# Joseph-93/PhotoHive_DSP

Measured on AMD Instinct MI355X. Metric: images/sec (4000×3000 RGB8 full report) at 1/2/4/8 GPUs; HBM GB/s vs peak, higher is better.
Workload: dtype f64

## Files before the change

### photohive_dsp_amd/csrc/fft_ct.hip

```cpp
#include <algorithm>
#include <cstdlib>

#pragma clang fp contract(fast)

#include "fft_engine.h"
#include "phd_device.h"

namespace phd {

namespace {

using namespace fe;

typedef unsigned u32x4 __attribute__((ext_vector_type(4)));

constexpr double kWr = 0.299 / 255.0, kWg = 0.587 / 255.0, kWb = 0.114 / 255.0;

typedef unsigned u32x3a __attribute__((ext_vector_type(3), aligned(4)));
typedef const __attribute__((address_space(1))) u32x3a gu32x3a;
#ifndef PHD_ROW_NT
#define PHD_ROW_NT 0
#endif

__device__ __forceinline__ int byte_of(const u32x3a& w, int b) {
    const unsigned x = (b >> 2) == 0 ? w.x : ((b >> 2) == 1 ? w.y : w.z);
    return (x >> (8 * (b & 3))) & 255;
}

__device__ __forceinline__ u32x3a rot_px(const u32x3a& w, int r) {
    const int b = 3 * r, q = b >> 2, sh = b & 3;
    const unsigned l0 = q == 0 ? w.x : (q == 1 ? w.y : w.z);
    const unsigned l1 = q == 0 ? w.y : (q == 1 ? w.z : w.x);
    const unsigned l2 = q == 0 ? w.z : (q == 1 ? w.x : w.y);
    u32x3a o;
    o.x = __builtin_amdgcn_alignbyte(l1, l0, (unsigned)sh);
    o.y = __builtin_amdgcn_alignbyte(l2, l1, (unsigned)sh);
    o.z = __builtin_amdgcn_alignbyte(l0, l2, (unsigned)sh);
    return o;
}

template <int E, bool HFULL>
__device__ __forceinline__ void walk_runs(const double* __restrict__ lgb, int r0, int rend, const unsigned* rl,
                                          unsigned sg, unsigned long long* sl, double bscale,
                                          const double2* __restrict__ lt) {
    auto flush = [&](int k, double m, int e) {
        const double acc = fmax((double)e * 0.69314718055994530942 + log_mant(m, lt), 0.0);
        atomicAdd(&sl[k], bin_fixed(acc, bscale));
    };
    if (r0 >= rend) return;
    const int idx = (int)(sg & 255u);
    const unsigned chm = sg >> 8;
    if (__all(__popc(chm) <= 2)) {
        const int f1 = __builtin_ctz(chm | 0x80000000u), f2 = __builtin_ctz((chm & (chm - 1)) | 0x80000000u);
        double mp = 1.0, m0 = 1.0, m1 = 1.0;
        int es = 0, e0 = 0, e1 = 0;
#pragma unroll
        for (int j = 0; j < E; j++) {
            const int r = r0 + j;
            if (HFULL || r < rend) {
                const double pv = lgb[r];
                if (j > 0) {
                    const bool c1 = f1 == j, c2 = f2 == j;
                    m0 = c1 ? mp : m0;
                    e0 = c1 ? es : e0;
                    m1 = c2 ? mp : m1;
                    e1 = c2 ? es : e1;
                    mp = (c1 || c2) ? 1.0 : mp;
                    es = (c1 || c2) ? 0 : es;
                }
                int e;
                mp *= frexp(pv, &e);
                es += e;
            }
        }
        const int n = __popc(chm);
        flush(idx, n == 0 ? mp : m0, n == 0 ? es : e0);
        if (n >= 1) flush(idx + 1, n == 1 ? mp : m1, n == 1 ? es : e1);
        if (n == 2) flush(idx + 2, mp, es);
        return;
    }
    unsigned q1 = rl[idx + 1], q2 = rl[min(idx + 2, kColRunsMax - 1)], q3 = rl[min(idx + 3, kColRunsMax - 1)];
    int qi = idx + 4;
    int cur = idx, nxt = (int)(q1 >> 16);
    int esum = 0, n = 0, b0 = 0, b1 = 0, e0 = 0, e1 = 0;
    double mp = 1.0;
    double m0 = 1.0, m1 = 1.0;
    auto close = [&]() {
        if (n == 0) {
            b0 = cur; m0 = mp; e0 = esum; n = 1;
        } else if (n == 1) {
            b1 = cur; m1 = mp; e1 = esum; n = 2;
        } else {
            flush(cur, mp, esum);
        }
    };
#pragma unroll
    for (int j = 0; j < E; j++) {
        const int r = r0 + j;
        if (HFULL || r < rend) {
            const double pv = lgb[r];
            if (r >= nxt) {
                close();
                cur++;
                q1 = q2;
                q2 = q3;
                q3 = rl[min(qi++, kColRunsMax - 1)];
                nxt = (int)(q1 >> 16);
                mp = 1.0;
                esum = 0;
            }
            int e;
            mp *= frexp(pv, &e);
            esum += e;
        }
    }
    close();
    if (n > 0) flush(b0, m0, e0);
    if (n > 1) flush(b1, m1, e1);
}

template <int W, int T, int... Rs>
struct RowK {
    static constexpr int NTW = tw_entries<1, Rs...>();
    static constexpr int G4 = W / 4;
    static constexpr int LR = (G4 + T - 1) / T;
    static constexpr size_t lds = sizeof(double2) * (W + NTW);
    static_assert(W % 4 == 0, "row plans need W % 4 == 0");
    static_assert(Radices<Rs...>::product == W, "plan");
    static constexpr int BPC = (int)((160 * 1024) / lds) < 2 ? (int)((160 * 1024) / lds) : 2;
    static constexpr int MINW = (T >= 512 ? 4 : 2) * BPC / 2 > 0 ? (T >= 512 ? 4 : 2) * BPC / 2 : 1;
};

template <int W, int T, int... Rs>
__global__ __launch_bounds__(T, (RowK<W, T, Rs...>::MINW)) void k_rows_ct(const uint8_t* __restrict__ img, int H,
                                               const unsigned long long* __restrict__ sums,
                                               const double* __restrict__ k255g, const double2* __restrict__ twg,
                                               double2* __restrict__ inter, int ablate_arg,
                                               unsigned long long* __restrict__ rsum,
                                               const uint8_t* const* __restrict__ imgs, int nimg, long istride) {
    using K = RowK<W, T, Rs...>;
    const int ablate = PHD_ABL(ablate_arg);
    extern __shared__ __attribute__((aligned(16))) unsigned char smem[];
    double2* buf = reinterpret_cast<double2*>(smem);
    double2* tw = buf + W;
    const int tid = threadIdx.x;
    for (int i = tid; i < K::NTW; i += T) tw[i] = twg[i];
    const int P = (H + 1) / 2, G = (P + 3) / 4;
    const int x = blockIdx.x & 7, q = blockIdx.x >> 3, QA = gridDim.x >> 5;
    const int a = q >> 2, i4 = q & 3;
    auto item = [&](int s, int& im, int& pr) {
        const int m = x + 8 * (a + s * QA);
        im = m / G;
        pr = 4 * (m - im * G) + i4;
        return im < nimg && pr < P;
    };

    u32x3a rg[K::LR][2];
    auto fetch = [&](int im, int pr) {
        const int y0 = 2 * pr;
        const uint8_t* r0 = (imgs ? imgs[im] : img) + (size_t)y0 * 3 * W;
        const uint8_t* r1 = (y0 + 1 < H) ? r0 + 3 * W : r0;
#pragma unroll
        for (int j = 0; j < K::LR; j++) {
            const int g = (K::G4 % T == 0 || tid + j * T < K::G4) ? tid + j * T : 0;
#if PHD_ROW_NT
            rg[j][0] = __builtin_nontemporal_load((gu32x3a*)(r0 + 12 * g));
            rg[j][1] = __builtin_nontemporal_load((gu32x3a*)(r1 + 12 * g));
#else
            rg[j][0] = *(gu32x3a*)(r0 + 12 * g);
            rg[j][1] = *(gu32x3a*)(r1 + 12 * g);
#endif
        }
    };
    int s = 0, im = 0, pr = 0;
    bool live = item(0, im, pr);
    if (live) fetch(im, pr);
    __syncthreads();
    unsigned cs[3] = {0u, 0u, 0u};
    const int rot = (tid >> 1) & 3;
    constexpr int WF_ = W / 2 + 1, KP_ = (WF_ + 1) / 2, NSO_ = (4 * KP_ + T - 1) / T;
    {
        double2* slot = inter + (size_t)P * ct_row_stride(W) + (blockIdx.x & 63) * NSO_;
#pragma unroll
        for (int j = 0; j < NSO_; j++)
            if ((4 * KP_) % T == 0 || tid + j * T < 4 * KP_) slot[j] = make_double2(0.0, 0.0);
    }
    auto step = [&]() __attribute__((always_inline)) {
        const int y0 = 2 * pr;
        const bool two = y0 + 1 < H;
#pragma unroll
        for (int j = 0; j < K::LR; j++) {
            const int g = tid + j * T;
            if (K::G4 % T == 0 || g < K::G4) {
                double2 z[4];
                const u32x3a w0 = rot_px(rg[j][0], rot), w1 = rot_px(rg[j][1], rot);
#pragma unroll
                for (int e = 0; e < 4; e++) {
                    const double p0 = kWr * byte_of(w0, 3 * e) + kWg * byte_of(w0, 3 * e + 1) +
                                      kWb * byte_of(w0, 3 * e + 2);
                    const double p1 = kWr * byte_of(w1, 3 * e) + kWg * byte_of(w1, 3 * e + 1) +
                                      kWb * byte_of(w1, 3 * e + 2);
                    z[e] = make_double2(p0, two ? p1 : 0.0);
                    if (rsum) {
                        cs[0] += byte_of(w0, 3 * e) + (two ? byte_of(w1, 3 * e) : 0);
                        cs[1] += byte_of(w0, 3 * e + 1) + (two ? byte_of(w1, 3 * e + 1) : 0);
                        cs[2] += byte_of(w0, 3 * e + 2) + (two ? byte_of(w1, 3 * e + 2) : 0);
                    }
                }
#pragma unroll
                for (int e = 0; e < 4; e++) buf[4 * g + ((e + rot) & 3)] = z[e];
            }
        }
        int imn, prn;
        const bool next = item(s + 1, imn, prn);
        if (!(ablate & 4)) fetch(next ? imn : im, next ? prn : pr);
        __syncthreads();
        if (!(ablate & 1)) fft_lds<W, T, 1, Rs...>(buf, tw, tid);
        constexpr int WF = W / 2 + 1, KP = (WF + 1) / 2;
        double2* orow = inter + ((ablate & 8) ? (size_t)(blockIdx.x & 7) * ct_row_stride(W)
                                              : im * istride + (size_t)pr * ct_row_stride(W));
        constexpr int NSO = (4 * KP + T - 1) / T;
#pragma unroll
        for (int j = 0; j < NSO; j++) {
            const int i = tid + j * T;
            if ((4 * KP) % T == 0 || i < 4 * KP) {
                if (ablate & 2) continue;
                const int k = 2 * (i >> 2) + ((i >> 1) & 1);
                const bool second = i & 1;
                const int kk = k < WF ? k : 0;
                const int e = second ? (kk == 0 ? 0 : W - kk) : kk;
                const double* zp = reinterpret_cast<const double*>(buf + e);
                const double A = zp[second ? 1 : 0], B = zp[second ? 0 : 1];
                const double Ap = dpp_pair_swap(A), Bp = dpp_pair_swap(B);
                const double f = (k < WF && (two || !second)) ? 0.5 : 0.0;
                orow[i] = make_double2(f * (A + Bp), f * (B - Ap));
            }
        }
        __syncthreads();
        s++;
        im = imn;
        pr = prn;
        live = next;
    };
    while (live) step();
    if (rsum) {
        unsigned long long* red = reinterpret_cast<unsigned long long*>(smem);
        unsigned long long w3[3];
#pragma unroll
        for (int c = 0; c < 3; c++) w3[c] = wave_sum((unsigned long long)cs[c]);
        if (lane_id() == 0)
#pragma unroll
            for (int c = 0; c < 3; c++) red[(tid >> 6) * 3 + c] = w3[c];
        __syncthreads();
        if (tid < 3) {
            unsigned long long t = 0;
            for (int w = 0; w < T / 64; w++) t += red[w * 3 + tid];
            if (t) atomicAdd(&rsum[tid], t);
        }
    }
}

template <int H, int T, bool FULL, int... Rs>
struct ColK {
    using PL = Plan<H, T, 1, Rs...>;
    using L = typename PL::Last;
    static constexpr int R = L::OUT;
    static constexpr int NTW = tw_entries<1, Rs...>();
    static constexpr int P = (H + 1) / 2;
    static constexpr int CR = (2 * P + T - 1) / T;
    static constexpr int E = (H + T - 1) / T;
    static constexpr int RPT = (kColRunsMax + T - 1) / T;
    static constexpr size_t lds_base =
        sizeof(double2) * (H + NTW + kLogTab) + (sizeof(unsigned) + sizeof(unsigned long long)) * kColRunsMax;
    static_assert(Radices<Rs...>::product == H, "plan");
    static_assert(T % 2 == 0, "threads cover whole row pairs");
    static_assert(H % 2 == 0, "column plans: whole row pairs (the half-prefetch split)");
    static constexpr int BPC1 = (int)((160 * 1024) / (sizeof(double2) * (H + NTW) + 1024)) < 2 ? 1 : 2;
#ifdef PHD_COL_MINW3
    static constexpr int MINW = (H == 3000 && !FULL) ? 3 : (T > 384 ? 4 : (T > 256 ? 3 : 2)) * BPC1 / 2;
#else
    static constexpr int MINW = (T > 384 ? 4 : (T > 256 ? 3 : 2)) * BPC1 / 2;
#endif
    static constexpr int WIDE = (0 + ... + ((Rs < 0 ? -Rs / 2 : Rs) >= 20 ? 1 : 0));
    static constexpr bool REMAT = MINW >= 3 || WIDE >= 2;
    static constexpr size_t lds_pf = lds_base + sizeof(double) * H;
    static constexpr bool PF = FULL && lds_pf * BPC1 <= 160 * 1024;
    static constexpr size_t lds = PF ? lds_pf : lds_base;
};

__device__ __forceinline__ void lds_dma16(const void* g, void* lds_wave_base) {
#if defined(__HIP_DEVICE_COMPILE__)
    const unsigned m = __builtin_amdgcn_readfirstlane(
        (unsigned)(uintptr_t)(__attribute__((address_space(3))) void*)lds_wave_base);
    unsigned keep;
    asm volatile("s_mov_b32 %0, m0\n\ts_mov_b32 m0, %2\n\ts_nop 0\n\tglobal_load_lds_dwordx4 %1, off\n\ts_mov_b32 m0, %0"
                 : "=&s"(keep)
                 : "v"(g), "s"(m)
                 : "memory");
#else
    (void)g;
    (void)lds_wave_base;
#endif
}

__device__ __forceinline__ void wait_vmem() { __builtin_amdgcn_s_waitcnt(0x0F70); }

template <int H, int T, bool FULL, int... Rs>
__global__ __launch_bounds__(T, (ColK<H, T, FULL, Rs...>::MINW)) void k_cols_ct(const double2* __restrict__ inter0, int wf,
                                                     const unsigned* __restrict__ runs,
                                                     const unsigned* __restrict__ segidx, int rstride,
                                                     unsigned long long* __restrict__ bin_sums0, double* __restrict__ fmax_part0,
                                                     const double2* __restrict__ twg,
                                                     const unsigned long long* __restrict__ sums0, int width,
                                                     double* __restrict__ dbg, double bscale, int ablate_arg,
                                                     int nimg, long istride, long bstride, long fstride, long sstride) {
    using K = ColK<H, T, FULL, Rs...>;
    const int ablate = PHD_ABL(ablate_arg);
    using L = typename K::L;
    constexpr int R = K::R;
    extern __shared__ __attribute__((aligned(16))) unsigned char smem[];
    double2* buf = reinterpret_cast<double2*>(smem);
    double2* tw = buf + H;
    double2* lt = tw + K::NTW;
    unsigned long long* sl = reinterpret_cast<unsigned long long*>(lt + kLogTab);
    unsigned* rl = reinterpret_cast<unsigned*>(sl + kColRunsMax);
    double* lgb = K::PF ? reinterpret_cast<double*>(rl + kColRunsMax) : reinterpret_cast<double*>(buf);
    const int tid0 = threadIdx.x;
    int tid = tid0;
    const double2* inter = inter0;
    unsigned long long* bin_sums = bin_sums0;
    double* fmax_part = fmax_part0;
    const unsigned long long* sums = sums0;
    const int quad = (int)((blockIdx.x >> 3) & 3);
    const int half = quad & 1;
    for (int i = tid; i < K::NTW; i += T) tw[i] = twg[i];
    for (int i = tid; i < kColRunsMax; i += T) sl[i] = 0ull;
    log_table_init(lt, tid, T);
    const int kpn = (wf + 1) / 2;
    const size_t rs = (size_t)((4 * kpn + 7) & ~7);
    const int nunit = (kpn + 1) / 2;
// ... 153 lines not shown
template <int H, int T, bool PF, int... Rs>
int cols_grid_form() {
    const int g = bpc_cap("PHD_COL_BPC", resident_grid(k_cols_ct<H, T, PF, Rs...>, T, ColK<H, T, PF, Rs...>::lds)) /
                  32 * 32;
    return g < 32 ? 32 : g;
}

template <int H, int T, int... Rs>
int cols_grid() {
    static const int g = [] {
        int a = cols_grid_form<H, T, false, Rs...>();
        if constexpr (ColK<H, T, true, Rs...>::PF) a = std::max(a, cols_grid_form<H, T, true, Rs...>());
        return a;
    }();
    return g;
}

template <int H, int T, bool PF, int... Rs>
hipError_t cols_ct_form(const double2* inter, int width, int wf, const ColBins& cb, unsigned long long* bin_sums,
                        double* fmax_part, const double2* tw, const unsigned long long* sums, double* dbg,
                        hipStream_t st, int nimg, long istride, long bstride, long fstride, long sstride) {
    static const int grid = cols_grid_form<H, T, PF, Rs...>();
    phd_launch((k_cols_ct<H, T, PF, Rs...>), dim3(grid), dim3(T), ColK<H, T, PF, Rs...>::lds, st, inter, wf,
               cb.runs, cb.seg, cb.rstride, bin_sums, fmax_part, tw, sums, width, dbg, bin_scale(H, wf), g_ablate,
               nimg, istride, bstride, fstride, sstride);
    return hipGetLastError();
}

template <int H, int T, int... Rs>
hipError_t cols_ct(const double2* inter, int width, int wf, const ColBins& cb, unsigned long long* bin_sums,
                   double* fmax_part, const double2* tw, const unsigned long long* sums, double* dbg,
                   hipStream_t st, bool pf, int nimg = 1, long istride = 0, long bstride = 0, long fstride = 0,
                   long sstride = 0) {
    if constexpr (ColK<H, T, true, Rs...>::PF) {
        if (pf)
            return cols_ct_form<H, T, true, Rs...>(inter, width, wf, cb, bin_sums, fmax_part, tw, sums, dbg, st,
                                                   nimg, istride, bstride, fstride, sstride);
    }
    return cols_ct_form<H, T, false, Rs...>(inter, width, wf, cb, bin_sums, fmax_part, tw, sums, dbg, st, nimg,
                                            istride, bstride, fstride, sstride);
}

__global__ __launch_bounds__(256) void k_log_mant(const double* __restrict__ x, double* __restrict__ y, long n) {
    __shared__ double2 lt[kLogTab];
    log_table_init(lt, threadIdx.x, 256);
    __syncthreads();
    const long i = (long)blockIdx.x * 256 + threadIdx.x;
    if (i < n) y[i] = log_mant(x[i], lt);
}

__global__ __launch_bounds__(320) void k_fft_split_test(const double2* __restrict__ x, const double2* __restrict__ twg,
                                                        double2* __restrict__ X) {
    constexpr int N = 3000, T = 320;
    using PL = Plan<N, T, 1, 15, 10, PHD_SPLIT(20)>;
    using L = typename PL::Last;
    constexpr int NTW = tw_entries<1, 15, 10, PHD_SPLIT(20)>();
    __shared__ __attribute__((aligned(16))) double2 buf[N];
    __shared__ __attribute__((aligned(16))) double2 tw[NTW];
    const int tid = threadIdx.x;
    const size_t base = (size_t)blockIdx.x * N;
    for (int i = tid; i < N; i += T) buf[i] = x[base + i];
    for (int i = tid; i < NTW; i += T) tw[i] = twg[i];
    __syncthreads();
    PL::template all_but_last<true>(buf, tw, tid);
    double2 v[L::ROUNDS][L::OUT];
    L::load(buf, v, tid);
    L::compute(v, tw + PL::last_tw_offset, tid);
#pragma unroll
    for (int q = 0; q < L::ROUNDS; q++) {
        const int b = L::row0(tid, q);
        if (L::active(tid, q)) {
#pragma unroll
            for (int k = 0; k < L::OUT; k++) X[base + b + k * L::NB] = v[q][k];
        }
    }
}

}

hipError_t launch_fft_split_test(const double2* x, const double2* tw, double2* X, int n, hipStream_t st) {
    if (n <= 0) return hipSuccess;
    phd_launch(k_fft_split_test, dim3((unsigned)n), dim3(320), 0, st, x, tw, X);
    return hipGetLastError();
}

hipError_t launch_log_mant(const double* x, double* y, long n, hipStream_t st) {
    if (n <= 0) return hipSuccess;
    phd_launch(k_log_mant, dim3((unsigned)((n + 255) / 256)), dim3(256), 0, st, x, y, n);
    return hipGetLastError();
}

bool ct_rows_plan(int w, std::vector<int>* radices) {
#define PHD_X(N, T, ...)                                       \
    if (w == N) {                                              \
        if (radices) *radices = std::vector<int>{__VA_ARGS__}; \
        return true;                                           \
    }
    PHD_CT_ROWS(PHD_X)
#undef PHD_X
    return false;
}

bool ct_cols_plan(int h, std::vector<int>* radices) {
#define PHD_X(N, T, ...)                                       \
    if (h == N) {                                              \
        if (radices) {                                         \
            *radices = std::vector<int>{__VA_ARGS__};          \
            for (int& r : *radices) r = std::abs(r);           \
        }                                                      \
        return true;                                           \
    }
    PHD_CT_COLS(PHD_X)
#undef PHD_X
    return false;
}

int fft_cols_ct_threads(int h) {
#define PHD_X(N, T, ...) \
    if (h == N) return T;
    PHD_CT_COLS(PHD_X)
#undef PHD_X
    return 0;
}

size_t fft_cols_ct_lds(int h) {
#define PHD_X(N, T, ...) \
    if (h == N) return ColK<N, T, false, __VA_ARGS__>::lds;
    PHD_CT_COLS(PHD_X)
#undef PHD_X
    return 0;
}

int fft_cols_ct_blocks(int h) {
#define PHD_X(N, T, ...) \
    if (h == N) return cols_grid<N, T, __VA_ARGS__>();
    PHD_CT_COLS(PHD_X)
#undef PHD_X
    return 0;
}

hipError_t launch_fft_rows_ct(const uint8_t* img, int height, int width, const unsigned long long* sums,
                              const double* k255, const double2* tw, double2* inter, hipStream_t st,
                              unsigned long long* rsum) {
#define PHD_X(N, T, ...) \
// ... 45 lines not shown
```

### photohive_dsp_amd/csrc/fft_engine.h

```cpp
#pragma once

#include <hip/hip_runtime.h>

#include <type_traits>
#include <utility>

#include "fft_consts.h"

namespace phd {
namespace fe {

#define PHD_HD __host__ __device__ __forceinline__

PHD_HD double2 cadd(double2 a, double2 b) { return make_double2(a.x + b.x, a.y + b.y); }
PHD_HD double2 csub(double2 a, double2 b) { return make_double2(a.x - b.x, a.y - b.y); }
PHD_HD double2 cmul(double2 a, double2 b) {
    return make_double2(a.x * b.x - a.y * b.y, a.x * b.y + a.y * b.x);
}
PHD_HD double2 mul_negi(double2 a) { return make_double2(a.y, -a.x); }
PHD_HD double2 mul_posi(double2 a) { return make_double2(-a.y, a.x); }

template <typename F, int... Is>
PHD_HD void sfor_impl(F&& f, std::integer_sequence<int, Is...>) {
    (f(std::integral_constant<int, Is>{}), ...);
}
template <int N, typename F>
PHD_HD void sfor(F&& f) {
    sfor_impl(f, std::make_integer_sequence<int, N>{});
}

template <int R, int M>
PHD_HD double2 twm(double2 a) {
    constexpr int m = M % R;
    constexpr double h = 0.70710678118654752440;
    if constexpr (m == 0) return a;
    else if constexpr (2 * m == R) return make_double2(-a.x, -a.y);
    else if constexpr (4 * m == R) return mul_negi(a);
    else if constexpr (4 * m == 3 * R) return mul_posi(a);
    else if constexpr (8 * m == R) return make_double2(h * (a.x + a.y), h * (a.y - a.x));
    else if constexpr (8 * m == 3 * R) return make_double2(h * (a.y - a.x), -h * (a.x + a.y));
    else if constexpr (8 * m == 5 * R) return make_double2(-h * (a.x + a.y), h * (a.x - a.y));
    else if constexpr (8 * m == 7 * R) return make_double2(h * (a.x - a.y), h * (a.x + a.y));
    else {
        constexpr double c = TwTab<R>::c[m], s = TwTab<R>::s[m];
        return make_double2(a.x * c + a.y * s, a.y * c - a.x * s);
    }
}

template <int R>
PHD_HD void dft(double2 (&v)[R]);

template <>
PHD_HD void dft<1>(double2 (&)[1]) {}

template <>
PHD_HD void dft<2>(double2 (&v)[2]) {
    const double2 a = v[0], b = v[1];
    v[0] = cadd(a, b);
    v[1] = csub(a, b);
}

template <>
PHD_HD void dft<3>(double2 (&v)[3]) {
    constexpr double s1 = 0.86602540378443864676;
    const double2 t = cadd(v[1], v[2]);
// ... 95 lines not shown
            constexpr int n1 = decltype(n1_)::value;
            y[n2][n1] = v[pfa_in<A, B>(n1, n2)];
        });
        dft<A>(y[n2]);
    });
    sfor<A>([&](auto k1_) {
        constexpr int k1 = decltype(k1_)::value;
        double2 z[B];
        sfor<B>([&](auto n2_) { z[decltype(n2_)::value] = y[decltype(n2_)::value][k1]; });
        dft<B>(z);
        sfor<B>([&](auto k2_) { v[pfa_out<A, B>(k1, decltype(k2_)::value)] = z[decltype(k2_)::value]; });
    });
}

#ifndef PHD_DFT_PFA
#define PHD_DFT_PFA 1
#endif
template <int R>
PHD_HD void dft(double2 (&v)[R]) {
    constexpr int A = split_of(R), B = R / A;
    if constexpr (PHD_DFT_PFA != 0 && gcd_of(A, B) == 1) dft_pfa<A, B>(v);
    else dft_ab<A, B>(v);
}

template <int M>
PHD_HD void split_twiddle(double2 (&v)[M], const double2 w, int h) {
    const double2 w2 = cmul(w, w), w4 = cmul(w2, w2), w8 = cmul(w4, w4);
    double2 p[4];
    p[0] = make_double2(h ? w.x : 1.0, h ? w.y : 0.0);
    p[1] = cmul(p[0], w2);
    p[2] = cmul(p[0], w4);
    p[3] = cmul(p[1], w4);
    sfor<M>([&](auto j_) {
        constexpr int j = decltype(j_)::value;
        if constexpr (j > 3) p[j & 3] = cmul(p[j & 3], w8);
        v[j] = cmul(v[j], p[j & 3]);
    });
}
template <int M>
PHD_HD void split_half(double2 (&v)[M], int h) {
    dft<M>(v);
    sfor<M>([&](auto k_) {
        constexpr int k = decltype(k_)::value;
        const double2 t = twm<2 * M, k>(v[k]);
        v[k] = make_double2(h ? t.x : v[k].x, h ? t.y : v[k].y);
    });
}
PHD_HD double2 split_join(double2 a, double2 p, int h) {
    const double s = h ? -1.0 : 1.0;
    return make_double2(p.x + s * a.x, p.y + s * a.y);
}

template <int R>
__device__ __forceinline__ void twiddle_powers(double2 (&v)[R], const double2 w) {
    if constexpr (R <= 4) {
        double2 wr = w;
        v[1] = cmul(v[1], w);
#pragma unroll
        for (int r = 2; r < R; r++) {
            wr = cmul(wr, w);
            v[r] = cmul(v[r], wr);
        }
    } else {
        double2 p[4];
        p[1] = w;
        p[2] = cmul(w, w);
        p[3] = cmul(p[2], w);
        p[0] = cmul(p[2], p[2]);
        const double2 w4 = p[0];
#pragma unroll
        for (int r = 1; r < R; r++) {
            if (r > 4) p[r & 3] = cmul(p[r & 3], w4);
            v[r] = cmul(v[r], p[r & 3]);
        }
    }
}

template <bool ON>
__device__ __forceinline__ int opaque(int x) {
    if constexpr (ON) asm volatile("" : "+v"(x));
    return x;
}

template <int N, int T, int R, int NS, bool CLAMP = false>
struct Pass {
    static constexpr int NB = N / R;
    static constexpr int ROUNDS = (NB + T - 1) / T;
    static constexpr bool FULL = NB % T == 0;
    static_assert(N % R == 0, "radix must divide N");

    static constexpr int OUT = R;
    __device__ static __forceinline__ bool active(int b) { return FULL || b < NB; }
    __device__ static __forceinline__ bool active(int tid, int q) { return active(tid + q * T); }
    __device__ static __forceinline__ int row0(int tid, int q) { return tid + q * T; }
    __device__ static __forceinline__ int bfly(int tid, int q) {
        return (FULL || !CLAMP) ? tid + q * T : min(tid + q * T, NB - 1);
    }

    __device__ static __forceinline__ void load(const double2* buf, double2 (&v)[ROUNDS][R], int tid) {
#pragma unroll
        for (int q = 0; q < ROUNDS; q++) {
            const int b = bfly(tid, q);
            if (CLAMP || active(b)) {
#pragma unroll
                for (int r = 0; r < R; r++) v[q][r] = buf[b + r * NB];
            }
        }
    }
    __device__ static __forceinline__ void compute(double2 (&v)[ROUNDS][R], const double2* tw, int tid) {
#pragma unroll
        for (int q = 0; q < ROUNDS; q++) {
            const int b = bfly(tid, q);
            if (CLAMP || active(b)) {
                if constexpr (NS > 1) twiddle_powers<R>(v[q], tw[b % NS]);
                dft<R>(v[q]);
            }
        }
    }
    __device__ static __forceinline__ void store(double2* buf, const double2 (&v)[ROUNDS][R], int tid) {
#pragma unroll
        for (int q = 0; q < ROUNDS; q++) {
            const int b = tid + q * T;
            if (active(b)) {
                const int jh = b / NS, jm = b - jh * NS;
                const int base = jh * NS * R + jm;
#pragma unroll
                for (int k = 0; k < R; k++) buf[base + k * NS] = v[q][k];
            }
        }
    }
};

__device__ __forceinline__ double dpp_pair_swap(double x) {
    const unsigned long long u = __builtin_bit_cast(unsigned long long, x);
    const unsigned lo = (unsigned)__builtin_amdgcn_mov_dpp((int)(unsigned)u, 0xB1, 0xF, 0xF, false);
    const unsigned hi = (unsigned)__builtin_amdgcn_mov_dpp((int)(unsigned)(u >> 32), 0xB1, 0xF, 0xF, false);
    return __builtin_bit_cast(double, ((unsigned long long)hi << 32) | lo);
}

template <int N, int T, int R, int NS>
struct SplitPass {
    static constexpr int M = R / 2;
    static constexpr int NB = N / R;
    static constexpr int ROUNDS = 1;
    static constexpr int OUT = M;
    static_assert(N % R == 0 && R % 2 == 0, "even radix dividing N");
    static_assert(2 * NB <= T && T % 2 == 0, "a split pass is one round of lane pairs");

    __device__ static __forceinline__ bool active(int tid, int) { return tid < 2 * NB; }
    __device__ static __forceinline__ int row0(int tid, int) { return (tid >> 1) + (tid & 1) * M * NB; }
    __device__ static __forceinline__ int bfly(int tid) { return min(tid >> 1, NB - 1); }

    __device__ static __forceinline__ void load(const double2* buf, double2 (&v)[ROUNDS][M], int tid) {
        const int b = bfly(tid), h = tid & 1;
#pragma unroll
        for (int j = 0; j < M; j++) v[0][j] = buf[b + (2 * j + h) * NB];
    }
    __device__ static __forceinline__ void compute(double2 (&v)[ROUNDS][M], const double2* tw, int tid) {
        const int b = bfly(tid), h = tid & 1;
        if constexpr (NS > 1) split_twiddle<M>(v[0], tw[b % NS], h);
        split_half<M>(v[0], h);
#pragma unroll
        for (int k = 0; k < M; k++) {
            const double2 p = make_double2(dpp_pair_swap(v[0][k].x), dpp_pair_swap(v[0][k].y));
            v[0][k] = split_join(v[0][k], p, h);
        }
    }
};

template <int... Rs>
struct Radices {
    static constexpr int count = sizeof...(Rs);
    static constexpr int product = (1 * ... * (Rs < 0 ? -Rs : Rs));
};

template <int NS, int R, int... Rest>
constexpr int tw_entries() {
    if constexpr (sizeof...(Rest) == 0) return NS > 1 ? NS : 0;
    else return (NS > 1 ? NS : 0) + tw_entries<NS * R, Rest...>();
}


template <int N, int T, int NS, int R, int... Rest>
__device__ __forceinline__ void fft_lds(double2* buf, const double2* tw, int tid) {
    using P = Pass<N, T, R, NS>;
    double2 v[P::ROUNDS][R];
    P::load(buf, v, tid);
    P::compute(v, tw, tid);
    __syncthreads();
    P::store(buf, v, tid);
    __syncthreads();
    if constexpr (sizeof...(Rest) > 0) fft_lds<N, T, NS * R, Rest...>(buf, tw + (NS > 1 ? NS : 0), tid);
}

#ifndef PHD_COL_CLAMP
#define PHD_COL_CLAMP 1
#endif
template <int N, int T, int NS, int R, int... Rest>
struct Plan {
    using Last = typename Plan<N, T, NS * R, Rest...>::Last;
    static constexpr int last_tw_offset = (NS > 1 ? NS : 0) + Plan<N, T, NS * R, Rest...>::last_tw_offset;
    template <bool REMAT = false>
    __device__ static __forceinline__ void all_but_last(double2* buf, const double2* tw, int tid0) {
        using P = Pass<N, T, R, NS, PHD_COL_CLAMP != 0>;
        const int tid = opaque<REMAT>(tid0);
        double2 v[P::ROUNDS][R];
        P::load(buf, v, tid);
        P::compute(v, tw, tid);
        __syncthreads();
        P::store(buf, v, tid);
        __syncthreads();
        Plan<N, T, NS * R, Rest...>::template all_but_last<REMAT>(buf, tw + (NS > 1 ? NS : 0), tid0);
    }
};
template <int N, int T, int NS, int R>
struct Plan<N, T, NS, R> {
    using Last = std::conditional_t<(R < 0), SplitPass<N, T, (R < 0 ? -R : 2), NS>, Pass<N, T, (R < 0 ? 1 : R), NS, PHD_COL_CLAMP != 0>>;
    static constexpr int last_tw_offset = 0;
    template <bool REMAT = false>
    __device__ static __forceinline__ void all_but_last(double2*, const double2*, int) {}
};

}
}
```

### photohive_dsp_amd/csrc/phd_context.cpp

```cpp
#include <atomic>
#include <cmath>
#include <cstdio>
#include <cstring>

#include <chrono>
#include <cstdlib>
#include <thread>

#include <unistd.h>

#include "phd_host.h"

namespace phd {

namespace {
void register_shutdown();
thread_local std::string g_error;
thread_local double g_timings[8];
thread_local int g_ntimings = 0;
std::mutex g_ctx_mu;
Context* g_ctx[64][kLanes] = {};
}

void set_error(const std::string& msg) {
    g_error = msg;
    if (!getenv("PHD_QUIET"))
        fprintf(stderr, "%s%s\n", msg.compare(0, 7, "Error: ") == 0 ? "" : "Error: ", msg.c_str());
}
void clear_error() { g_error.clear(); }

void record_timings(const double* ms, int n) {
    g_ntimings = n < 8 ? n : 8;
    for (int i = 0; i < g_ntimings; i++) g_timings[i] = ms[i];
}

Context* get_context() { return get_context_lane(0); }

Context* get_context_lane(int lane) {
    int dev = -1;
    if (hipGetDevice(&dev) != hipSuccess || dev < 0 || dev >= 64) {
        int n = 0;
        if (hipGetDeviceCount(&n) != hipSuccess || n <= 0) {
            set_error("no HIP device available: the MI355X path has no CPU fallback");
            return nullptr;
        }
        dev = 0;
        if (hipSetDevice(0) != hipSuccess) {
            set_error("hipSetDevice(0) failed");
            return nullptr;
        }
    }
    std::lock_guard<std::mutex> lk(g_ctx_mu);
    if (g_ctx[dev][lane]) return g_ctx[dev][lane];
    register_shutdown();
    auto* c = new Context();
    c->device = dev;
    c->pid = getpid();
    if (hipStreamCreateWithFlags(&c->stream, hipStreamNonBlocking) != hipSuccess) {
        set_error("hipStreamCreate failed");
        delete c;
        return nullptr;
    }
    double k255[256];
// ... 188 lines not shown
        else f += 2;
    }
    if (m != 1) {
        set_error("FFT length " + std::to_string(n) + " has too many factors");
        return false;
    }
    P.generic = 0;
    P.composite = 0;
    for (int i = 0; i < P.npass; i++) {
        const int r = P.radix[i];
        const bool comp = r == 6 || r == 9 || r == 10 || r == 12 || r == 16;
        if (r != 2 && r != 3 && r != 4 && r != 5 && r != 8 && !comp) P.generic = 1;
        P.composite |= comp ? 1 : 0;
    }
    P.n_hi = (n + 63) / 64;
    const long double two_pi = 6.283185307179586476925286766559005768L;
    auto w = [&](long t) {
        const long double a = two_pi * (long double)(t % n) / (long double)n;
        return make_double2((double)cosl(a), (double)-sinl(a));
    };
    std::vector<double2> tw(n + 64 + P.n_hi);
    for (int t = 0; t < n; t++) tw[t] = w(t);
    for (int t = 0; t < 64; t++) tw[n + t] = w(t);
    for (int t = 0; t < P.n_hi; t++) tw[n + 64 + t] = w(64L * t);
    if (hipMalloc(&p->d_tw, sizeof(double2) * tw.size()) != hipSuccess ||
        hipMemcpy(p->d_tw, tw.data(), sizeof(double2) * tw.size(), hipMemcpyHostToDevice) != hipSuccess) {
        set_error("twiddle upload failed");
        return false;
    }
    P.tw = p->d_tw;
    P.tw_lo = p->d_tw + n;
    P.tw_hi = p->d_tw + n + 64;
    return true;
}

const FftPlanHost* get_plan(Context* c, int n, bool composite) {
    const auto key = std::make_pair(n, composite);
    auto it = c->plans.find(key);
    if (it != c->plans.end()) return &it->second;
    FftPlanHost p;
    if (!make_fft_plan(n, &p, composite)) return nullptr;
    return &(c->plans[key] = p);
}

const double2* get_ct_twiddles(Context* c, int n, bool rows) {
    const auto key = std::make_pair(n, rows ? 1 : 0);
    auto it = c->ct_tw.find(key);
    if (it != c->ct_tw.end()) return it->second;
    std::vector<int> rad;
    if (!(rows ? ct_rows_plan(n, &rad) : ct_cols_plan(n, &rad))) {
        set_error("no compile-time FFT plan for length " + std::to_string(n));
        return nullptr;
    }
    const long double two_pi = 6.283185307179586476925286766559005768L;
    std::vector<double2> tw;
    long ns = 1;
    for (int r : rad) {
        if (ns > 1)
            for (long jm = 0; jm < ns; jm++) {
                const long double a = two_pi * (long double)jm / (long double)(ns * r);
                tw.push_back(make_double2((double)cosl(a), (double)-sinl(a)));
            }
        ns *= r;
    }
    if (tw.empty()) tw.push_back(make_double2(1.0, 0.0));
    double2* d = nullptr;
    if (hipMalloc(&d, sizeof(double2) * tw.size()) != hipSuccess ||
        hipMemcpy(d, tw.data(), sizeof(double2) * tw.size(), hipMemcpyHostToDevice) != hipSuccess) {
        set_error("compile-time FFT twiddle upload failed");
        return nullptr;
    }
    c->ct_tw[key] = d;
    return d;
}

namespace {
#ifndef PHD_COLUMN_FORM
#define PHD_COLUMN_FORM -1
#endif
std::atomic<int> g_column_form{PHD_COLUMN_FORM};
}

int FftSel::forced_form() { return g_column_form.load(std::memory_order_relaxed); }

bool select_fft(Context* c, int height, int width, int nbins, const uint8_t* const* imgs, int n, FftSel* s,
                const BlurTable* tbl, bool batch) {
    *s = FftSel{};
    if (FftSel::forced_form() >= 0) s->col_pf = FftSel::forced_form() == 1;
    static const bool force_generic = phd_knob("PHD_FFT_GENERIC") != nullptr;
    bool ct = !force_generic && ct_rows_plan(width, nullptr) && ct_cols_plan(height, nullptr) &&
              fft_cols_ct_lds(height) <= 160 * 1024;
    for (int i = 0; ct && i < n; i++)
        if (reinterpret_cast<uintptr_t>(imgs[i]) & 3) ct = false;
    const ColRuns* runs = nullptr;
    if (ct && tbl) {
        const int T = fft_cols_ct_threads(height);
        (void)batch;
        {
            const auto key = std::make_tuple(height, width, tbl->nr, tbl->na, T);
            auto f = c->colruns.find(key);
            if (f == c->colruns.end()) {
                ColRuns r;
                if (build_col_runs(tbl->map.data(), tbl->height, tbl->wf, T, &r) || r.too_many)
                    f = c->colruns.emplace(key, r).first;
            }
            if (f != c->colruns.end() && f->second.d_runs) runs = &f->second;
            else ct = false;
        }
    }
    if (ct) {
        s->ct = true;
        s->tw_r = get_ct_twiddles(c, width, true);
        s->tw_c = get_ct_twiddles(c, height, false);
        if (!s->tw_r || !s->tw_c) return false;
        s->cbins = ColBins{runs ? runs->d_runs : nullptr, runs ? runs->d_seg : nullptr, runs ? runs->stride : 0};
        s->col_blocks = fft_cols_ct_blocks(height);
        return true;
// ... 386 lines not shown
```

### photohive_dsp_amd/csrc/phd_internal.h

```cpp
#pragma once

#include <hip/hip_runtime_api.h>
#include <stddef.h>
#include <stdint.h>
#include <stdlib.h>

#include <vector>

#include "sharp_tiles.h"

namespace phd {

inline const char* phd_knob(const char* name) {
#ifdef PHD_ABLATE_BUILD
    return getenv(name);
#else
    (void)name;
    return nullptr;
#endif
}

struct LaunchEvents {
    hipEvent_t start = nullptr, stop = nullptr;
    bool used = false;
// ... 130 lines not shown
hipError_t launch_palette_sums(const uint8_t* img, int height, int width, int ds,
                               const GridParams& gp, const GroupRule* rules,
                               const double* slot_off, int nslots, double* out,
                               const double* k255, hipStream_t st);
hipError_t launch_fft_rows_batch(const uint8_t* const* d_imgs, int n, int height, int width, const FftPlan& plan,
                                 const unsigned long long* sums0, long sums_stride, const double* k255,
                                 double2* inter0, size_t inter_stride, hipStream_t st);
hipError_t launch_fft_cols_batch(const double2* inter0, size_t inter_stride, int n, int height, int wf,
                                 const FftPlan& plan, const uint16_t* binmap, int nbins, unsigned long long* bin_sums0,
                                 double* fmax_part0, long out_stride, hipStream_t st);
hipError_t launch_fft_rows(const uint8_t* img, int height, int width, const FftPlan& plan,
                           const unsigned long long* sums, const double* k255,
                           double2* inter, hipStream_t st);
hipError_t launch_fft_cols(const double2* inter, int height, int wf, const FftPlan& plan,
                           const uint16_t* binmap, int nbins, unsigned long long* bin_sums,
                           double* fmax_part, hipStream_t st, double bscale = 0.0);
int fft_cols_blocks(int height, int wf, int nbins, const FftPlan& plan, size_t* lds, int* lds_bins);

#define PHD_CT_ROWS(X)           \
    X(4000, 512, 5, 8, 10, 10)   \
    X(6000, 512, 6, 10, 10, 10)  \
    X(3000, 384, 5, 6, 10, 10)   \
    X(2000, 256, 5, 4, 10, 10)   \
     \
    X(2048, 256, 8, 16, 16)      \
    X(1920, 256, 15, 8, 16)      \
    X(1280, 256, 5, 16, 16)      \
    X(720, 192, 5, 9, 16)        \
    X(640, 128, 5, 8, 16)        \
    X(480, 128, 5, 6, 16)        \
    X(512, 64, 8, 8, 8)
#define PHD_SPLIT(R) (-(R))
#ifndef PHD_C3000_T
#define PHD_C3000_T 256
#endif
#ifndef PHD_C3000_R
#define PHD_C3000_R 15, 10, 20
#endif
#define PHD_CT_COLS(X)           \
    X(3000, PHD_C3000_T, PHD_C3000_R) \
    X(6000, 512, 15, 20, 20)     \
    X(4000, 256, 10, 20, 20)     \
    X(2000, 256, 10, 10, 20)     \
     \
    X(1536, 256, 3, 8, 8, 8)     \
    X(1080, 192, 15, 8, 9)       \
    X(1280, 256, 5, 16, 16)      \
    X(720, 192, 5, 9, 16)        \
    X(640, 128, 5, 8, 16)        \
    X(480, 128, 5, 6, 16)        \
    X(512, 64, 8, 8, 8)
bool ct_rows_plan(int w, std::vector<int>* radices);
bool ct_cols_plan(int h, std::vector<int>* radices);
constexpr int ct_row_stride(int width) { return (4 * (((width / 2 + 1) + 1) / 2) + 7) & ~7; }
inline size_t inter_elems(int height, int width) {
    const size_t generic = (size_t)(height + 1) * (width / 2 + 2);
    const size_t ct = (size_t)((height + 1) / 2) * ct_row_stride(width);
    return (generic > ct ? generic : ct) + 1024;
}
constexpr int kColRunsMax = 256;
struct ColBins {
    const uint32_t* runs = nullptr;
    const uint32_t* seg = nullptr;
    int rstride = 0;
};
size_t fft_cols_ct_lds(int height);
int fft_cols_ct_threads(int height);
hipError_t launch_log_mant(const double* x, double* y, long n, hipStream_t st);
hipError_t launch_fft_split_test(const double2* x, const double2* tw, double2* X, int n, hipStream_t st);
int fft_cols_ct_blocks(int height);
hipError_t launch_fft_rows_ct(const uint8_t* img, int height, int width, const unsigned long long* sums,
                              const double* k255, const double2* tw, double2* inter, hipStream_t st,
                              unsigned long long* rsum = nullptr);
hipError_t launch_fft_cols_ct(const double2* inter, int height, int width, int wf, const ColBins& cb,
                              unsigned long long* bin_sums, double* fmax_part, const double2* tw,
                              const unsigned long long* sums, double* dbg, hipStream_t st, bool pf = true);
hipError_t launch_fft_rows_ct_batch(const uint8_t* const* d_imgs, int n, int height, int width, const double* k255,
                                    const double2* tw, double2* inter, long inter_stride, hipStream_t st);
hipError_t launch_fft_cols_ct_batch(const double2* inter, long inter_stride, int n, int height, int width, int wf,
                                    const ColBins& cb, unsigned long long* bin_sums, long bin_stride,
                                    double* fmax_part, long fmax_stride, const double2* tw,
                                    const unsigned long long* sums, long sums_stride, hipStream_t st,
                                    bool pf = true);
struct KernelProfiler;
int prof_begin_sharp(KernelProfiler* prof, hipStream_t st);
void prof_end(KernelProfiler* prof, int slot, hipStream_t st);
hipError_t launch_sharpness_src(const uint8_t* img, const double* pgm, int height, int width, int n, const int* top,
                                const int* bottom, const int* left, const int* right, const double* k255,
                                double* sums, hipStream_t st, KernelProfiler* prof = nullptr);
hipError_t launch_sharpness_batch(const uint8_t* const* d_imgs, const SharpBox* d_boxes, const int* d_prefix,
                                  int nboxes, int nslices, int width, const double* k255, SharpPart* d_parts,
                                  double* out0, long out_stride, hipStream_t st, KernelProfiler* prof = nullptr);

struct PackRec;
int prof_begin_pack(KernelProfiler* prof, hipStream_t st);
hipError_t launch_pack_views(const PackRec* d_recs, int n, int max_bands, hipStream_t st,
                             KernelProfiler* prof = nullptr);

struct DecodeRec;
constexpr int kProfClassify = 7, kProfDecode = 8;
int prof_begin_kernel(KernelProfiler* prof, int kernel, hipStream_t st);
hipError_t launch_classify_views(const DecodeRec* d_recs, int* d_flags, int n, int max_bands, hipStream_t st,
                                 KernelProfiler* prof = nullptr);
hipError_t launch_decode_view(const DecodeRec& rec, hipStream_t st, KernelProfiler* prof = nullptr);

struct PlanarSrc {
// ... 40 lines not shown
```

Before: 10340.

## Compute luma with integer dot4 and add optional full twiddle tables

```diff
diff --git a/photohive_dsp_amd/csrc/fft_ct.hip b/photohive_dsp_amd/csrc/fft_ct.hip
--- a/photohive_dsp_amd/csrc/fft_ct.hip
+++ b/photohive_dsp_amd/csrc/fft_ct.hip
@@ -4,6 +4,7 @@
 #pragma clang fp contract(fast)
 
 #include "fft_engine.h"
+#include "luma_int.h"
 #include "phd_device.h"
 
 namespace phd {
@@ -14,7 +15,14 @@
 
 typedef unsigned u32x4 __attribute__((ext_vector_type(4)));
 
+#ifndef PHD_LUMA_INT
+#define PHD_LUMA_INT 1
+#endif
+#if PHD_LUMA_INT
+constexpr double kLumaHalf = 0.5 / kLumaDen;
+#else
 constexpr double kWr = 0.299 / 255.0, kWg = 0.587 / 255.0, kWb = 0.114 / 255.0;
+#endif
 
 typedef unsigned u32x3a __attribute__((ext_vector_type(3), aligned(4)));
 typedef const __attribute__((address_space(1))) u32x3a gu32x3a;
@@ -121,12 +129,17 @@
 
 template <int W, int T, int... Rs>
 struct RowK {
-    static constexpr int NTW = tw_entries<1, Rs...>();
+    static constexpr int rad[] = {Rs...};
+    static constexpr unsigned FM = tw_full_mask(rad, (int)sizeof...(Rs), (long)sizeof(double2) * W, T);
+    static constexpr int NTW = tw_entries<FM, 0, 1, Rs...>();
+    static constexpr int NTW0 = tw_entries<0u, 0, 1, Rs...>();
     static constexpr int G4 = W / 4;
     static constexpr int LR = (G4 + T - 1) / T;
     static constexpr size_t lds = sizeof(double2) * (W + NTW);
     static_assert(W % 4 == 0, "row plans need W % 4 == 0");
     static_assert(Radices<Rs...>::product == W, "plan");
+    static_assert(lds_blocks((long)lds, T) == lds_blocks((long)sizeof(double2) * (W + NTW0), T),
+                  "the twiddle tables must not lower the blocks per CU");
     static constexpr int BPC = (int)((160 * 1024) / lds) < 2 ? (int)((160 * 1024) / lds) : 2;
     static constexpr int MINW = (T >= 512 ? 4 : 2) * BPC / 2 > 0 ? (T >= 512 ? 4 : 2) * BPC / 2 : 1;
 };
@@ -188,6 +201,9 @@
     auto step = [&]() __attribute__((always_inline)) {
         const int y0 = 2 * pr;
         const bool two = y0 + 1 < H;
+#if PHD_LUMA_INT
+        const double lum1 = two ? kLumaHalf : 0.0;
+#endif
 #pragma unroll
         for (int j = 0; j < K::LR; j++) {
             const int g = tid + j * T;
@@ -196,11 +212,17 @@
                 const u32x3a w0 = rot_px(rg[j][0], rot), w1 = rot_px(rg[j][1], rot);
 #pragma unroll
                 for (int e = 0; e < 4; e++) {
+#if PHD_LUMA_INT
+                    const double p0 = luma_from_int(luma_int(group_px(w0.x, w0.y, w0.z, e)), kLumaHalf);
+                    const double p1 = luma_from_int(luma_int(group_px(w1.x, w1.y, w1.z, e)), lum1);
+                    z[e] = make_double2(p0, p1);
+#else
                     const double p0 = kWr * byte_of(w0, 3 * e) + kWg * byte_of(w0, 3 * e + 1) +
                                       kWb * byte_of(w0, 3 * e + 2);
                     const double p1 = kWr * byte_of(w1, 3 * e) + kWg * byte_of(w1, 3 * e + 1) +
                                       kWb * byte_of(w1, 3 * e + 2);
                     z[e] = make_double2(p0, two ? p1 : 0.0);
+#endif
                     if (rsum) {
                         cs[0] += byte_of(w0, 3 * e) + (two ? byte_of(w1, 3 * e) : 0);
                         cs[1] += byte_of(w0, 3 * e + 1) + (two ? byte_of(w1, 3 * e + 1) : 0);
@@ -215,11 +237,12 @@
         const bool next = item(s + 1, imn, prn);
         if (!(ablate & 4)) fetch(next ? imn : im, next ? prn : pr);
         __syncthreads();
-        if (!(ablate & 1)) fft_lds<W, T, 1, Rs...>(buf, tw, tid);
+        if (!(ablate & 1)) fft_lds<W, T, K::FM, 0, 1, Rs...>(buf, tw, tid);
         constexpr int WF = W / 2 + 1, KP = (WF + 1) / 2;
         double2* orow = inter + ((ablate & 8) ? (size_t)(blockIdx.x & 7) * ct_row_stride(W)
                                               : im * istride + (size_t)pr * ct_row_stride(W));
         constexpr int NSO = (4 * KP + T - 1) / T;
+        auto stores = [&](const bool odd) __attribute__((always_inline)) {
 #pragma unroll
         for (int j = 0; j < NSO; j++) {
             const int i = tid + j * T;
@@ -232,10 +255,28 @@
                 const double* zp = reinterpret_cast<const double*>(buf + e);
                 const double A = zp[second ? 1 : 0], B = zp[second ? 0 : 1];
                 const double Ap = dpp_pair_swap(A), Bp = dpp_pair_swap(B);
-                const double f = (k < WF && (two || !second)) ? 0.5 : 0.0;
+#if PHD_LUMA_INT
+                double re = A + Bp, im = B - Ap;
+                const bool phantom = WF % 2 == 1 && (j + 1) * T > 2 * WF;
+                if (phantom || odd) {
+                    const bool zero = (phantom && k >= WF) || (odd && second);
+                    re = zero ? 0.0 : re;
+                    im = zero ? 0.0 : im;
+                }
+                orow[i] = make_double2(re, im);
+#else
+                const double f = (k < WF && (!odd || !second)) ? 0.5 : 0.0;
                 orow[i] = make_double2(f * (A + Bp), f * (B - Ap));
+#endif
             }
         }
+        };
+#if PHD_LUMA_INT
+        if (two) stores(false);
+        else stores(true);
+#else
+        stores(!two);
+#endif
         __syncthreads();
         s++;
         im = imn;
@@ -262,10 +303,18 @@
 
 template <int H, int T, bool FULL, int... Rs>
 struct ColK {
-    using PL = Plan<H, T, 1, Rs...>;
+    static constexpr int rad[] = {abs_radix(Rs)...};
+    static constexpr int NTW0 = tw_entries<0u, 0, 1, Rs...>();
+    static constexpr long lds_fixed =
+        (long)sizeof(double2) * (H + kLogTab) + (long)(sizeof(unsigned) + sizeof(unsigned long long)) * kColRunsMax;
+    static constexpr int BPC1 = (int)((160 * 1024) / (sizeof(double2) * (H + NTW0) + 1024)) < 2 ? 1 : 2;
+    static constexpr bool PF0 = (lds_fixed + (long)sizeof(double2) * NTW0 + (long)sizeof(double) * H) * BPC1 <= 160 * 1024;
+    static constexpr unsigned FM =
+        H == 512 ? 0u : tw_full_mask(rad, (int)sizeof...(Rs), lds_fixed + (PF0 ? (long)sizeof(double) * H : 0), T);
+    using PL = Plan<H, T, FM, 0, 1, Rs...>;
     using L = typename PL::Last;
     static constexpr int R = L::OUT;
-    static constexpr int NTW = tw_entries<1, Rs...>();
+    static constexpr int NTW = tw_entries<FM, 0, 1, Rs...>();
     static constexpr int P = (H + 1) / 2;
     static constexpr int CR = (2 * P + T - 1) / T;
     static constexpr int E = (H + T - 1) / T;
@@ -275,17 +324,22 @@
     static_assert(Radices<Rs...>::product == H, "plan");
     static_assert(T % 2 == 0, "threads cover whole row pairs");
     static_assert(H % 2 == 0, "column plans: whole row pairs (the half-prefetch split)");
-    static constexpr int BPC1 = (int)((160 * 1024) / (sizeof(double2) * (H + NTW) + 1024)) < 2 ? 1 : 2;
 #ifdef PHD_COL_MINW3
     static constexpr int MINW = (H == 3000 && !FULL) ? 3 : (T > 384 ? 4 : (T > 256 ? 3 : 2)) * BPC1 / 2;
 #else
     static constexpr int MINW = (T > 384 ? 4 : (T > 256 ? 3 : 2)) * BPC1 / 2;
 #endif
+    static constexpr int REGB = MINW * 4 / ((T + 63) / 64) > 0 ? MINW * 4 / ((T + 63) / 64) : 1;
+    static_assert(lds_blocks((long)lds_base, T) >= lds_blocks(lds_fixed + 16L * NTW0, T) ||
+                      lds_blocks((long)lds_base, T) >= REGB,
+                  "the twiddle tables must not lower the half-prefetch form's blocks per CU");
     static constexpr int WIDE = (0 + ... + ((Rs < 0 ? -Rs / 2 : Rs) >= 20 ? 1 : 0));
     static constexpr bool REMAT = MINW >= 3 || WIDE >= 2;
     static constexpr size_t lds_pf = lds_base + sizeof(double) * H;
     static constexpr bool PF = FULL && lds_pf * BPC1 <= 160 * 1024;
     static constexpr size_t lds = PF ? lds_pf : lds_base;
+    static_assert(PF == (FULL && PF0), "the twiddle tables must not cost the plan its full-prefetch form");
+    static_assert(lds * BPC1 <= 160 * 1024, "the twiddle tables must not lower the blocks per CU");
 };
 
 __device__ __forceinline__ void lds_dma16(const void* g, void* lds_wave_base) {
@@ -545,9 +599,10 @@
 __global__ __launch_bounds__(320) void k_fft_split_test(const double2* __restrict__ x, const double2* __restrict__ twg,
                                                         double2* __restrict__ X) {
     constexpr int N = 3000, T = 320;
-    using PL = Plan<N, T, 1, 15, 10, PHD_SPLIT(20)>;
+    constexpr unsigned FM = ColK<3000, PHD_C3000_T, false, PHD_C3000_R>::FM;
+    using PL = Plan<N, T, FM, 0, 1, 15, 10, PHD_SPLIT(20)>;
     using L = typename PL::Last;
-    constexpr int NTW = tw_entries<1, 15, 10, PHD_SPLIT(20)>();
+    constexpr int NTW = tw_entries<FM, 0, 1, 15, 10, PHD_SPLIT(20)>();
     __shared__ __attribute__((aligned(16))) double2 buf[N];
     __shared__ __attribute__((aligned(16))) double2 tw[NTW];
     const int tid = threadIdx.x;
@@ -583,6 +638,18 @@
     return hipGetLastError();
 }
 
+unsigned ct_tw_full_mask(int n, bool rows) {
+#define PHD_X(N, T, ...) \
+    if (rows && n == N) return RowK<N, T, __VA_ARGS__>::FM;
+    PHD_CT_ROWS(PHD_X)
+#undef PHD_X
+#define PHD_X(N, T, ...) \
+    if (!rows && n == N) return ColK<N, T, false, __VA_ARGS__>::FM;
+    PHD_CT_COLS(PHD_X)
+#undef PHD_X
+    return 0u;
+}
+
 bool ct_rows_plan(int w, std::vector<int>* radices) {
 #define PHD_X(N, T, ...)                                       \
     if (w == N) {                                              \
diff --git a/photohive_dsp_amd/csrc/fft_engine.h b/photohive_dsp_amd/csrc/fft_engine.h
--- a/photohive_dsp_amd/csrc/fft_engine.h
+++ b/photohive_dsp_amd/csrc/fft_engine.h
@@ -6,11 +6,11 @@
 #include <utility>
 
 #include "fft_consts.h"
+#include "fft_twtab.h"
 
 namespace phd {
 namespace fe {
 
-#define PHD_HD __host__ __device__ __forceinline__
 
 PHD_HD double2 cadd(double2 a, double2 b) { return make_double2(a.x + b.x, a.y + b.y); }
 PHD_HD double2 csub(double2 a, double2 b) { return make_double2(a.x - b.x, a.y - b.y); }
@@ -212,7 +212,7 @@
 }
 
 template <int R>
-__device__ __forceinline__ void twiddle_powers(double2 (&v)[R], const double2 w) {
+PHD_HD void twiddle_powers(double2 (&v)[R], const double2 w) {
     if constexpr (R <= 4) {
         double2 wr = w;
         v[1] = cmul(v[1], w);
@@ -236,13 +236,21 @@
     }
 }
 
+template <int R, int NS>
+PHD_HD void twiddle_powers(double2 (&v)[R], const double2* tab, int jm) {
+    sfor<R - 1>([&](auto r_) {
+        constexpr int r = decltype(r_)::value + 1;
+        v[r] = cmul(v[r], tab[tw_index(NS, r, jm)]);
+    });
+}
+
 template <bool ON>
 __device__ __forceinline__ int opaque(int x) {
     if constexpr (ON) asm volatile("" : "+v"(x));
     return x;
 }
 
-template <int N, int T, int R, int NS, bool CLAMP = false>
+template <int N, int T, int R, int NS, bool CLAMP = false, bool TAB = false>
 struct Pass {
     static constexpr int NB = N / R;
     static constexpr int ROUNDS = (NB + T - 1) / T;
@@ -272,7 +280,8 @@
         for (int q = 0; q < ROUNDS; q++) {
             const int b = bfly(tid, q);
             if (CLAMP || active(b)) {
-                if constexpr (NS > 1) twiddle_powers<R>(v[q], tw[b % NS]);
+                if constexpr (NS > 1 && TAB) twiddle_powers<R, NS>(v[q], tw, b % NS);
+                else if constexpr (NS > 1) twiddle_powers<R>(v[q], tw[b % NS]);
                 dft<R>(v[q]);
             }
         }
@@ -334,35 +343,39 @@
     static constexpr int product = (1 * ... * (Rs < 0 ? -Rs : Rs));
 };
 
-template <int NS, int R, int... Rest>
+constexpr int abs_radix(int r) { return r < 0 ? -r : r; }
+template <unsigned FM, int PI, int NS, int R, int... Rest>
 constexpr int tw_entries() {
-    if constexpr (sizeof...(Rest) == 0) return NS > 1 ? NS : 0;
-    else return (NS > 1 ? NS : 0) + tw_entries<NS * R, Rest...>();
-}
-
-
-template <int N, int T, int NS, int R, int... Rest>
+    constexpr int here = tw_pass_entries(abs_radix(R), NS, (FM >> PI) & 1u);
+    if constexpr (sizeof...(Rest) == 0) return here;
+    else return here + tw_entries<FM, PI + 1, NS * abs_radix(R), Rest...>();
+}
+
+template <int N, int T, unsigned FM, int PI, int NS, int R, int... Rest>
 __device__ __forceinline__ void fft_lds(double2* buf, const double2* tw, int tid) {
-    using P = Pass<N, T, R, NS>;
+    using P = Pass<N, T, R, NS, false, ((FM >> PI) & 1u) != 0>;
     double2 v[P::ROUNDS][R];
     P::load(buf, v, tid);
     P::compute(v, tw, tid);
     __syncthreads();
     P::store(buf, v, tid);
     __syncthreads();
-    if constexpr (sizeof...(Rest) > 0) fft_lds<N, T, NS * R, Rest...>(buf, tw + (NS > 1 ? NS : 0), tid);
+    if constexpr (sizeof...(Rest) > 0)
+        fft_lds<N, T, FM, PI + 1, NS * R, Rest...>(buf, tw + tw_pass_entries(R, NS, (FM >> PI) & 1u), tid);
 }
 
 #ifndef PHD_COL_CLAMP
 #define PHD_COL_CLAMP 1
 #endif
-template <int N, int T, int NS, int R, int... Rest>
+template <int N, int T, unsigned FM, int PI, int NS, int R, int... Rest>
 struct Plan {
-    using Last = typename Plan<N, T, NS * R, Rest...>::Last;
-    static constexpr int last_tw_offset = (NS > 1 ? NS : 0) + Plan<N, T, NS * R, Rest...>::last_tw_offset;
+    static constexpr bool TAB = ((FM >> PI) & 1u) != 0;
+    using Next = Plan<N, T, FM, PI + 1, NS * R, Rest...>;
+    using Last = typename Next::Last;
+    static constexpr int last_tw_offset = tw_pass_entries(R, NS, TAB) + Next::last_tw_offset;
     template <bool REMAT = false>
     __device__ static __forceinline__ void all_but_last(double2* buf, const double2* tw, int tid0) {
-        using P = Pass<N, T, R, NS, PHD_COL_CLAMP != 0>;
+        using P = Pass<N, T, R, NS, PHD_COL_CLAMP != 0, TAB>;
         const int tid = opaque<REMAT>(tid0);
         double2 v[P::ROUNDS][R];
         P::load(buf, v, tid);
@@ -370,12 +383,13 @@
         __syncthreads();
         P::store(buf, v, tid);
         __syncthreads();
-        Plan<N, T, NS * R, Rest...>::template all_but_last<REMAT>(buf, tw + (NS > 1 ? NS : 0), tid0);
-    }
-};
-template <int N, int T, int NS, int R>
-struct Plan<N, T, NS, R> {
-    using Last = std::conditional_t<(R < 0), SplitPass<N, T, (R < 0 ? -R : 2), NS>, Pass<N, T, (R < 0 ? 1 : R), NS, PHD_COL_CLAMP != 0>>;
+        Next::template all_but_last<REMAT>(buf, tw + tw_pass_entries(R, NS, TAB), tid0);
+    }
+};
+template <int N, int T, unsigned FM, int PI, int NS, int R>
+struct Plan<N, T, FM, PI, NS, R> {
+    using Last = std::conditional_t<(R < 0), SplitPass<N, T, (R < 0 ? -R : 2), NS>,
+                                    Pass<N, T, (R < 0 ? 1 : R), NS, PHD_COL_CLAMP != 0, ((FM >> PI) & 1u) != 0>>;
     static constexpr int last_tw_offset = 0;
     template <bool REMAT = false>
     __device__ static __forceinline__ void all_but_last(double2*, const double2*, int) {}
diff --git a/photohive_dsp_amd/csrc/fft_twtab.h b/photohive_dsp_amd/csrc/fft_twtab.h
--- /dev/null
+++ b/photohive_dsp_amd/csrc/fft_twtab.h
@@ -0,0 +1,84 @@
+#pragma once
+
+#include <hip/hip_runtime.h>
+
+#include <cmath>
+#include <vector>
+
+#ifndef PHD_HD
+#define PHD_HD __host__ __device__ __forceinline__
+#endif
+
+#ifndef PHD_TW_TABLES
+#define PHD_TW_TABLES 0
+#endif
+
+namespace phd {
+namespace fe {
+
+constexpr long kLdsPerCu = 160 * 1024;
+
+PHD_HD constexpr int tw_pass_entries(int R, int NS, bool full) { return NS > 1 ? (full ? (R - 1) * NS : NS) : 0; }
+PHD_HD constexpr int tw_index(int NS, int r, int jm) { return (r - 1) * NS + jm; }
+
+PHD_HD constexpr int lds_blocks(long lds, int threads) {
+    const int waves = (threads + 63) / 64, cap = 32 / waves > 0 ? 32 / waves : 1;
+    const long b = lds > 0 ? kLdsPerCu / lds : cap;
+    return b < cap ? (int)b : cap;
+}
+
+PHD_HD constexpr unsigned tw_full_mask(const int* rad, int passes, long fixed, int threads) {
+    long cur = 0;
+    int ns = 1;
+    for (int p = 0; p < passes; p++) {
+        cur += tw_pass_entries(rad[p], ns, false);
+        ns *= rad[p];
+    }
+    const int target = lds_blocks(fixed + 16 * cur, threads);
+    unsigned mask = 0;
+    ns = 1;
+    for (int p = 0; p < passes; p++) {
+        const long extra = tw_pass_entries(rad[p], ns, true) - tw_pass_entries(rad[p], ns, false);
+        if (PHD_TW_TABLES != 0 && ns > 1 && target > 0 && lds_blocks(fixed + 16 * (cur + extra), threads) == target) {
+            mask |= 1u << p;
+            cur += extra;
+        }
+        ns *= rad[p];
+    }
+    return mask;
+}
+
+PHD_HD constexpr int tw_plan_offset(const int* rad, int p, unsigned mask) {
+    int off = 0, ns = 1;
+    for (int q = 0; q < p; q++) {
+        off += tw_pass_entries(rad[q], ns, (mask >> q) & 1u);
+        ns *= rad[q];
+    }
+    return off;
+}
+PHD_HD constexpr int tw_plan_entries(const int* rad, int passes, unsigned mask) {
+    return tw_plan_offset(rad, passes, mask);
+}
+
+inline std::vector<double2> tw_build_table(const std::vector<int>& rad, unsigned mask) {
+    const long double two_pi = 6.283185307179586476925286766559005768L;
+    const int passes = (int)rad.size();
+    std::vector<double2> tab((size_t)tw_plan_entries(rad.data(), passes, mask));
+    long ns = 1;
+    for (int p = 0; p < passes; p++) {
+        const int R = rad[p];
+        const bool full = (mask >> p) & 1u;
+        double2* t = tab.data() + tw_plan_offset(rad.data(), p, mask);
+        if (ns > 1)
+            for (int r = 1; r < (full ? R : 2); r++)
+                for (long jm = 0; jm < ns; jm++) {
+                    const long double a = two_pi * (long double)(jm * r) / (long double)(ns * R);
+                    t[tw_index((int)ns, r, (int)jm)] = make_double2((double)cosl(a), (double)-sinl(a));
+                }
+        ns *= R;
+    }
+    return tab;
+}
+
+}
+}
diff --git a/photohive_dsp_amd/csrc/luma_int.h b/photohive_dsp_amd/csrc/luma_int.h
--- /dev/null
+++ b/photohive_dsp_amd/csrc/luma_int.h
@@ -0,0 +1,40 @@
+#pragma once
+
+#include <hip/hip_runtime.h>
+
+#ifndef PHD_HD
+#define PHD_HD __host__ __device__ __forceinline__
+#endif
+
+namespace phd {
+
+PHD_HD unsigned dot4_u8(unsigned a, unsigned b, unsigned c) {
+#if defined(__HIP_DEVICE_COMPILE__)
+    return __builtin_amdgcn_udot4(a, b, c, false);
+#else
+    for (int i = 0; i < 4; i++) c += ((a >> (8 * i)) & 255u) * ((b >> (8 * i)) & 255u);
+    return c;
+#endif
+}
+
+PHD_HD unsigned align_bytes(unsigned hi, unsigned lo, unsigned sh) {
+#if defined(__HIP_DEVICE_COMPILE__)
+    return __builtin_amdgcn_alignbyte(hi, lo, sh);
+#else
+    return (unsigned)(((((unsigned long long)hi) << 32) | lo) >> (8 * (sh & 3u)));
+#endif
+}
+
+PHD_HD unsigned luma_int(unsigned px) {
+    constexpr unsigned w0 = 44u | (77u << 8) | (114u << 16), w1 = 255u | (255u << 8), w2 = 255u << 8;
+    return dot4_u8(px, w0, dot4_u8(px, w1, dot4_u8(px, w2, 0u)));
+}
+
+PHD_HD unsigned group_px(unsigned x, unsigned y, unsigned z, int e) {
+    return e == 0 ? x : (e == 1 ? align_bytes(y, x, 3u) : (e == 2 ? align_bytes(z, y, 2u) : z >> 8));
+}
+
+constexpr double kLumaDen = 255000.0;
+PHD_HD double luma_from_int(unsigned L, double scale_over_den) { return (double)L * scale_over_den; }
+
+}
diff --git a/photohive_dsp_amd/csrc/phd_context.cpp b/photohive_dsp_amd/csrc/phd_context.cpp
--- a/photohive_dsp_amd/csrc/phd_context.cpp
+++ b/photohive_dsp_amd/csrc/phd_context.cpp
@@ -9,6 +9,7 @@
 
 #include <unistd.h>
 
+#include "fft_twtab.h"
 #include "phd_host.h"
 
 namespace phd {
@@ -303,17 +304,7 @@
         set_error("no compile-time FFT plan for length " + std::to_string(n));
         return nullptr;
     }
-    const long double two_pi = 6.283185307179586476925286766559005768L;
-    std::vector<double2> tw;
-    long ns = 1;
-    for (int r : rad) {
-        if (ns > 1)
-            for (long jm = 0; jm < ns; jm++) {
-                const long double a = two_pi * (long double)jm / (long double)(ns * r);
-                tw.push_back(make_double2((double)cosl(a), (double)-sinl(a)));
-            }
-        ns *= r;
-    }
+    std::vector<double2> tw = fe::tw_build_table(rad, ct_tw_full_mask(n, rows));
     if (tw.empty()) tw.push_back(make_double2(1.0, 0.0));
     double2* d = nullptr;
     if (hipMalloc(&d, sizeof(double2) * tw.size()) != hipSuccess ||
diff --git a/photohive_dsp_amd/csrc/phd_internal.h b/photohive_dsp_amd/csrc/phd_internal.h
--- a/photohive_dsp_amd/csrc/phd_internal.h
+++ b/photohive_dsp_amd/csrc/phd_internal.h
@@ -206,6 +206,7 @@
     X(512, 64, 8, 8, 8)
 bool ct_rows_plan(int w, std::vector<int>* radices);
 bool ct_cols_plan(int h, std::vector<int>* radices);
+unsigned ct_tw_full_mask(int n, bool rows);
 constexpr int ct_row_stride(int width) { return (4 * (((width / 2 + 1) + 1) / 2) + 7) & ~7; }
 inline size_t inter_elems(int height, int width) {
     const size_t generic = (size_t)(height + 1) * (width / 2 + 2);
```

New measurement: 10420 (median of 6 runs). Within noise of the previous version (+0.7%).
